# IllyaArtemchuk/Harmonies-Alphazero

Hardware: AMD Instinct MI355X
Metric: self-play env-steps/sec + games/sec @4096 boards, 1/2/4/8 GPUs; bit-exact vs CPU (higher is better)
Workload: dtype u64; 1 GPU; config2: 4096 concurrent boards/GPU, reset + rule-driven play to game end (legal mask, step, chance draws, final scoring); one step = 256 hz_play launches of 4096 boards; boards_per_gpu=4096, parallelism=shard1

## Files before the change

harmonies-alphazero_amd/csrc/hz_env.hip:

```cpp
#include <hip/hip_runtime.h>

#include <cstdio>
#include <cstdlib>
#include <cstring>

#include "../../include/hz_abi.h"
#include "hz_device.hpp"
#include "hz_encode.hpp"
#include "hz_host.hpp"

using namespace hz;
using namespace hz_host;

struct P2Draw {
  int32_t *tag;
  int32_t *k;
  uint64_t *q;
  uint64_t *bag;
  int32_t *c;
};
struct P2Mid {
  int32_t *tag;
  uint64_t *st;
  uint64_t *q;
  int32_t *i;
};

#ifndef HZ_P2_NDRAW
#define HZ_P2_NDRAW 5
#endif
#ifndef HZ_P2_NPLAY
#define HZ_P2_NPLAY 5
#endif
constexpr int kP2Draw = HZ_P2_NDRAW;
constexpr int kP2Play = HZ_P2_NPLAY;
constexpr int kP2SDraw = 4;
constexpr int kP2SPlay = kP2SDraw + kP2Draw;
constexpr int kP2Stages = kP2SPlay + kP2Play;
constexpr int kP2Last = kP2Stages - 1;
constexpr int kP2Ring = kP2Play + 1;
constexpr int kP2Stream = kP2Stages;
static_assert(kP2Draw >= 2 && kP2Draw <= 5 && kP2Play >= 2 && kP2Play <= 5, "stage counts");

struct hz_env {
  DevBufs bufs, p2_bufs, ar_bufs;
  int32_t n;
  uint64_t seed_base;
  hipStream_t stream;
  uint64_t *state;
  uint32_t *mt;
  int32_t *pos;
  int32_t *ply;
  int32_t *episode;
  uint64_t *seed;
  int seed_ahead;
  uint32_t *ahead_mt[2];
  int32_t *ahead_tag[2];
  uint64_t *ahead_pile[2];
  int32_t *ahead_cur[2];
  uint32_t *ahead_rule[2];
  int32_t *ep_final[2];
  size_t nrow;
  uint32_t *ring_mt[3];
  int32_t *ring_tag[3];
  uint64_t *ring_pile[3];
  int32_t *ring_cur[3];
  int32_t *ring_k1[3];
  int calls;
  int primed, slot_valid[2];
  int32_t *mt_src;
  int lazy;
  int ar_ahead;
  uint32_t *ar_mt;
  int32_t *ar_tag;
  uint64_t *ar_pile;
  int32_t *ar_cur;
  int32_t *ar_ep[2];
  int ar_calls, ar_primed;
  uint32_t *pw_words;
  int32_t *pw_tag;
  int pipeline;
  int calls2, primed2;
  int p2_cut[kP2Play - 1];
  int p2_dcut[kP2Draw + 1];
  int p2_fell_lim;
  uint32_t *p2_s[kP2Stream];
  int32_t *p2_s_tag[kP2Stream];
  int32_t *p2_s_cur[kP2Stream];
  uint32_t *p2_p1h[2];
  int32_t *p2_p1t[2];
  uint32_t *p2_p2h[2];
  uint32_t *p2_p3h[2];
  P2Draw p2_x[kP2Draw - 1][2];
  P2Draw p2_pl[kP2Ring];
  P2Mid p2_m[kP2Play - 1][2];
  uint32_t *p2_h[kP2Ring];
  int32_t *p2_h_tag[kP2Ring];
  int32_t *p2_ep[2];
  int32_t *wait_err_own;
  int32_t *wait_err;
  int spin_limit;
};

#ifdef HZ_DIAG
__device__ uint64_t *g_stamps;
__device__ int g_role_only = -1;
#define HZ_STAMP(slot)                                                    \
  do {                                                                    \
    __builtin_amdgcn_sched_barrier(0);                                    \
    if (g_stamps) g_stamps[(size_t)b * 16 + (slot)] = __builtin_amdgcn_s_memtime(); \
    __builtin_amdgcn_sched_barrier(0);                                    \
  } while (0)
#ifndef HZ_DIAG_ROLES_ONLY
#define HZ_ACC(slot, t0)                                                  \
  do {                                                                    \
    __builtin_amdgcn_sched_barrier(0);                                    \
    uint64_t _t = __builtin_amdgcn_s_memtime();                           \
    acc##slot += _t - (t0);                                               \
    t0 = _t;                                                              \
    __builtin_amdgcn_sched_barrier(0);                                    \
  } while (0)
#else
#define HZ_ACC(slot, t0) \
  do {                   \
  } while (0)
#endif
#define HZ_PHASE(slot, t0, b)                                                                 \
  do {                                                                                        \
    __builtin_amdgcn_sched_barrier(0);                                                        \
    if (g_stamps) g_stamps[(size_t)(b) * 16 + (slot)] = __builtin_amdgcn_s_memtime() - (t0); \
// ... 387 lines not shown
    if (lane + 64 * k < kMT) to[lane + 64 * k] = v[k];
  if (lane == 0) mt_src[b] = -1;
}

static PlyWin ply_win(hz_env *e) { return PlyWin{e->pw_words, e->pw_tag, (long)e->nrow}; }

static int touch(hz_env *e) { return streams_touched<HipDev>(e) ? 0 : 1; }

static int materialize(hz_env *e) {
  if (!e->lazy) return 0;
  if (e->ar_mt)
    hipLaunchKernelGGL(k_mt_materialize_ar, dim3(e->n), dim3(64), 0, e->stream, e->mt, e->ar_mt, e->mt_src, e->n);
  hipLaunchKernelGGL(k_mt_materialize, dim3(e->n), dim3(64), 0, e->stream, e->mt, e->ahead_mt[0], e->ahead_mt[1],
                     e->mt_src, e->n);
  if (e->p2_s[0])
    hipLaunchKernelGGL(k_mt_materialize2, dim3(grid_for(e->n)), dim3(kStageThreads), kResetLds, e->stream, e->mt,
                       e->seed, e->pos, e->mt_src, e->n);
  e->lazy = 0;
  return launch_err();
}

static_assert(sizeof(((hz_env *)0)->p2_s) / sizeof(uint32_t *) == kP2Stream, "slot ring");

static int p2_clear_tags(hz_env *e) {
  const size_t bytes = e->nrow * sizeof(int32_t);
  auto c = [&](int32_t *t) { return hipMemsetAsync(t, 0xff, bytes, e->stream) != hipSuccess; };
  for (int k = 0; k < kP2Stream; k++)
    if (c(e->p2_s_tag[k])) return 1;
  for (int k = 0; k < 2; k++)
    if (c(e->p2_p1t[k])) return 1;
  for (int k = 0; k < kP2Draw - 1; k++)
    if (c(e->p2_x[k][0].tag) || c(e->p2_x[k][1].tag)) return 1;
  for (int k = 0; k < kP2Ring; k++)
    if (c(e->p2_pl[k].tag) || c(e->p2_h_tag[k])) return 1;
  for (int k = 0; k < kP2Play - 1; k++)
    if (c(e->p2_m[k][0].tag) || c(e->p2_m[k][1].tag)) return 1;
  return 0;
}

static int alloc_p2(hz_env *e) {
  if (e->p2_s[0]) return 0;
  const size_t nr = e->nrow;
  DevBufs &o = e->p2_bufs;
  for (int k = 0; k < kP2Stream; k++) {
    o.get(e->p2_s[k], nr * kMT * 4);
    o.get(e->p2_s_tag[k], nr * 4);
    o.get(e->p2_s_cur[k], (kAheadDraws + 1) * nr * 4);
  }
  auto md = [&](P2Draw &d) {
    o.get(d.tag, nr * 4);
    o.get(d.k, nr * 4);
    o.get(d.q, kAheadWords * nr * 8);
    o.get(d.bag, nr * 8);
    o.get(d.c, nr * 4);
  };
  for (int k = 0; k < kP2Draw - 1; k++) md(e->p2_x[k][0]), md(e->p2_x[k][1]);
  for (int k = 0; k < kP2Ring; k++) {
    md(e->p2_pl[k]);
    o.get(e->p2_h[k], kRulePlies * nr * 4);
    o.get(e->p2_h_tag[k], nr * 4);
  }
  for (int k = 0; k < kP2Play - 1; k++)
    for (int j = 0; j < 2; j++) {
      P2Mid &mm = e->p2_m[k][j];
      o.get(mm.tag, nr * 4);
      o.get(mm.st, 6 * nr * 8);
      o.get(mm.q, 4 * nr * 8);
      o.get(mm.i, 3 * nr * 4);
    }
  for (int k = 0; k < 2; k++) {
    o.get(e->p2_p1h[k], nr * 4);
    o.get(e->p2_p1t[k], nr * 4);
    o.get(e->p2_p2h[k], 4 * nr * 4);
    o.get(e->p2_p3h[k], 4 * nr * 4);
    o.get(e->p2_ep[k], nr * 4);
  }
  if (!o.ok || p2_clear_tags(e)) {
    o.release();
    return 1;
  }
  e->primed2 = 0;
  return 0;
}

static int launch_play2(hz_env *e, int32_t max_plies, int32_t *games_done, int32_t *steps_done) {
  if (alloc_p2(e)) return 1;
  const int c = e->calls2, r = c & 1, w = r ^ 1;
  if (!e->primed2) {
    if (hipMemcpyAsync(e->p2_ep[w], e->episode, (size_t)e->n * sizeof(int32_t), hipMemcpyDeviceToDevice,
                       e->stream))
      return 1;
    e->primed2 = 1;
  }
  P2Args a{};
  a.st = e->state;
  a.mt = e->mt;
  a.pos = e->pos;
  a.ply = e->ply;
  a.episode = e->episode;
  a.seed = e->seed;
  a.n = e->n;
  a.max_plies = max_plies;
  a.err = e->wait_err;
  a.spin = e->spin_limit;
  a.seed_base = e->seed_base;
  a.nrow = (long)e->nrow;
  a.games_done = games_done;
  a.steps_done = steps_done;
  a.mt_src = e->mt_src;
  a.win_tag = e->pw_tag;
  a.ep_in = e->p2_ep[w];
  a.ep_out = e->p2_ep[r];
  auto sl = [c](int s) { return ((c - s) % kP2Stream + kP2Stream) % kP2Stream; };
  for (int s = 1; s < kP2SDraw; s++) {
    a.s_mt[s] = e->p2_s[sl(s)];
    a.s_tag[s] = e->p2_s_tag[sl(s)];
  }
  a.s_idx_last = sl(kP2Last);
  a.p1h_w = e->p2_p1h[r];
  a.p1t_w = e->p2_p1t[r];
  a.p2h_w = e->p2_p2h[r];
  a.p3h_w = e->p2_p3h[r];
  a.seed_tag[0] = e->p2_p1t[w];
  a.seed_tag[1] = a.s_tag[2];
  a.seed_tag[2] = a.s_tag[3];
  a.seed_h[0] = e->p2_p1h[w];
  a.seed_h[1] = e->p2_p2h[w];
  a.seed_h[2] = e->p2_p3h[w];
  const int draws = e->seed_ahead;
  for (int k = 0; k < kP2Draw; k++) {
    P2DrawArgs &d = a.dr[k];
    const int s = kP2SDraw + k;
    d.slot = e->p2_s[sl(s)];
    d.stag = e->p2_s_tag[sl(s)];
    d.cur = e->p2_s_cur[sl(s)];
    d.in = e->p2_x[k > 0 ? k - 1 : 0][w];
    d.out = k == kP2Draw - 1 ? e->p2_pl[c % kP2Ring] : e->p2_x[k][r];
    d.d0 = e->p2_dcut[k];
    d.d1 = k == kP2Draw - 1 ? draws : std::min(draws, e->p2_dcut[k + 1]);
  }
  a.h_w = e->p2_h[c % kP2Ring];
  a.ht_w = e->p2_h_tag[c % kP2Ring];
  for (int st = 0; st < kP2Play; st++) {
    P2PlayArgs &p = a.pp[st];
    const bool last = st == kP2Play - 1;
    const int s = kP2SPlay + st;
    const int k = (c + kP2Ring - 1 - st) % kP2Ring;
    p.ep = last ? e->episode : e->p2_ep[w];
    p.ep_off = last ? 0 : kP2Play - 1 - st;
    p.g0 = st > 0 ? e->p2_cut[st - 1] : 0;
    p.g_end = last ? max_plies : std::min(e->p2_cut[st], max_plies);
    p.fell_lim = e->p2_fell_lim;
    p.ptag = e->p2_pl[k].tag;
    p.pk = e->p2_pl[k].k;
    p.q = st > 0 ? e->p2_m[st - 1][w].q : e->p2_pl[k].q;
    p.h = e->p2_h[k];
    p.ht = e->p2_h_tag[k];
    p.slot = e->p2_s[sl(s)];
    p.cur = e->p2_s_cur[sl(s)];
    p.in = e->p2_m[st > 0 ? st - 1 : 0][w];
    p.out = e->p2_m[last ? 0 : st][r];
  }
  const int nblk = grid_for(e->n);
  hipLaunchKernelGGL(k_play2, dim3(4 * nblk), dim3(kStageThreads), kResetLds, e->stream, a, nblk);
  if (int err = launch_err()) return err;
  e->lazy = 1;
  e->calls2 = (c + 1) % (kP2Stream * kP2Ring * 2);
  e->primed = 0;
  e->ar_primed = 0;
  return 0;
}

extern "C" {

hz_env *hz_env_create(int32_t n_boards, uint64_t seed_base, void *stream) {
  if (n_boards <= 0) return nullptr;
  if (install_comp_table()) return nullptr;
  if (lds_opt_in<k_reset>(kResetLds) || lds_opt_in<k_rollout<false, false>>(kResetLds) ||
      lds_opt_in<k_rollout<false, true>>(kResetLds) || lds_opt_in<k_rollout<true, false>>(kResetLds) ||
      lds_opt_in<k_rollout<true, true>>(kResetLds) || lds_opt_in<k_play2>(kResetLds) ||
      lds_opt_in<k_mt_materialize2>(kResetLds))
    return nullptr;
  hz_env *e = new (std::nothrow) hz_env();
  if (!e) return nullptr;
  e->n = n_boards;
  e->seed_base = seed_base;
  e->stream = (hipStream_t)stream;
  const size_t n = (size_t)n_boards, nr = (n + kBlock - 1) / kBlock * kBlock, i32 = sizeof(int32_t);
  e->nrow = nr;
  DevBufs &o = e->bufs;
  o.get(e->state, n * 6 * sizeof(uint64_t), 0);
  o.get(e->mt, n * 624 * sizeof(uint32_t));
  o.get(e->pos, n * i32, 0);
  o.get(e->ply, n * i32, 0);
  o.get(e->episode, n * i32, 0);
  o.get(e->seed, n * sizeof(uint64_t), 0);
  o.get(e->mt_src, n * i32, 0xff);
  for (int k = 0; k < 2; k++) {
    o.get(e->ahead_mt[k], n * kMT * sizeof(uint32_t));
    o.get(e->ahead_tag[k], n * i32, 0xff);
    o.get(e->ahead_pile[k], n * kAheadWords * sizeof(uint64_t));
    o.get(e->ahead_cur[k], n * (kAheadDraws + 1) * i32);
    o.get(e->ahead_rule[k], nr * kRulePlies * sizeof(uint32_t));
    o.get(e->ep_final[k], n * i32);
  }
  for (int k = 0; k < kRing; k++) {
    o.get(e->ring_mt[k], nr * kMT * sizeof(uint32_t));
    o.get(e->ring_tag[k], nr * i32, 0xff);
    o.get(e->ring_pile[k], nr * 3 * sizeof(uint64_t));
    o.get(e->ring_cur[k], nr * (kD1Draws + 1) * i32);
    o.get(e->ring_k1[k], nr * i32);
  }
  o.get(e->pw_words, nr * kPlyWin * sizeof(uint32_t));
  o.get(e->pw_tag, nr * i32, 0xff);
  o.get(e->wait_err_own, i32, 0);
  e->seed_ahead = kAheadDraws;
  e->ar_ahead = env_pick("HZ_AR_AHEAD", 0, 1);
  e->pipeline = env_pick("HZ_PIPELINE", 1, 2);
  for (int k = 0; k < kP2Play - 1; k++) e->p2_cut[k] = kP2PCut[k];
  if constexpr (kP2Play == 4) env_cuts("HZ_P2_CUTS", e->p2_cut);
  else if constexpr (kP2Play == 5) env_cuts_n("HZ_P2_CUTS5", e->p2_cut, kP2Play - 1, 4, 1 << 20);
  for (int k = 0; k < kP2Draw; k++) e->p2_dcut[k] = kP2DCut[k];
  e->p2_dcut[kP2Draw] = kAheadDraws;
  if constexpr (kP2Draw == 5) {
    int dc[kP2Draw + 1];
    for (int k = 0; k <= kP2Draw; k++) dc[k] = e->p2_dcut[k];
    if (env_cuts_n("HZ_P2_DCUTS", dc + 1, kP2Draw - 1, 1, kAheadDraws - 1) &&
        cuts_gaps_within(dc, kP2Draw + 1, kP2StageDraws))
      for (int k = 0; k <= kP2Draw; k++) e->p2_dcut[k] = dc[k];
  }
  e->p2_fell_lim = env_clamped("HZ_P2_FELL_LIMIT", kP2Twist, 0, kP2Twist);
  e->wait_err = e->wait_err_own;
  e->spin_limit = kSpinLimitDefault;
  if (!o.ok || hipDeviceSynchronize() != hipSuccess) {
    hz_env_destroy(e);
    return nullptr;
  }
  return e;
}

void hz_env_destroy(hz_env *e) {
  if (!e) return;
  e->p2_bufs.release();
  e->ar_bufs.release();
  e->bufs.release();
  delete e;
}

int32_t hz_env_size(const hz_env *e) { return e ? e->n : -1; }

int hz_env_set_error_word(hz_env *e, int32_t *word) {
  if (!e) return -1;
  e->wait_err = word ? word : e->wait_err_own;
  return 0;
}

int hz_env_set_spin_limit(hz_env *e, int32_t limit) {
  if (!e || limit < 0) return -1;
  e->spin_limit = limit ? limit : kSpinLimitDefault;
  return 0;
}

int hz_env_set_pipeline(hz_env *e, int32_t pipeline) {
// ... 302 lines not shown
```

harmonies-alphazero_amd/csrc/hz_host.hpp:

```cpp
#pragma once

#include <atomic>
#include <cstddef>
#include <cstdint>
#include <cstdio>
#include <cstdlib>
#include <new>
#include <vector>

namespace hz_host {

inline int env_int(const char *name, int dflt) {
  const char *e = getenv(name);
  return e ? atoi(e) : dflt;
}

inline int env_pick(const char *name, int special, int otherwise) {
  return env_int(name, otherwise) == special ? special : otherwise;
}

inline int env_clamped(const char *name, int dflt, int lo, int hi) {
  const int v = env_int(name, dflt);
  return v < lo ? lo : v > hi ? hi : v;
}

inline void env_cuts(const char *name, int cut[3]) {
  const char *e = getenv(name);
  int c[3];
  if (e && sscanf(e, "%d,%d,%d", &c[0], &c[1], &c[2]) == 3 && c[0] > 0 && c[1] > c[0] && c[2] > c[1] &&
      c[0] % 4 == 0 && c[1] % 4 == 0 && c[2] % 4 == 0)
    for (int k = 0; k < 3; k++) cut[k] = c[k];
}

inline bool env_cuts_n(const char *name, int *cut, int n, int step, int hi) {
  const char *e = getenv(name);
  if (!e || n < 1 || n > 8 || step < 1) return false;
  int c[8];
  for (int k = 0; k < n; k++) {
    if (*e < '0' || *e > '9') return false;
    long v = 0;
    for (; *e >= '0' && *e <= '9'; e++)
      if ((v = v * 10 + (*e - '0')) > hi) return false;
    if (v < step || v % step || (k && v <= c[k - 1])) return false;
    c[k] = (int)v;
    if (*e++ != (k + 1 < n ? ',' : '\0')) return false;
  }
  for (int k = 0; k < n; k++) cut[k] = c[k];
  return true;
}

inline bool cuts_gaps_within(const int *cut, int n, int max_gap) {
  for (int k = 0; k + 1 < n; k++)
    if (cut[k + 1] - cut[k] > max_gap) return false;
  return true;
}

struct Setting {
  static constexpr int64_t kUnread = INT64_MIN;
  const char *name;
  int32_t dflt;
  std::atomic<int64_t> v{kUnread};
  int32_t get() {
    int64_t x = v.load(std::memory_order_relaxed);
    if (x == kUnread) {
      int64_t expect = kUnread;
      v.compare_exchange_strong(expect, (int64_t)env_int(name, dflt));
      x = v.load(std::memory_order_relaxed);
    }
    return (int32_t)x;
  }
  void set(int32_t x) { v.store(x, std::memory_order_relaxed); }
};

template <class Dev>
struct DevBufsT {
  struct Held {
    void *p;
    void *slot;
    void (*clear)(void *slot);
  };
  std::vector<Held> held;
  bool ok = true;

  template <class T>
  bool get(T *&p, size_t bytes) {
    if (!ok) return false;
// ... 68 lines not shown
```

harmonies-alphazero_amd/csrc/hz_play2.hpp:

```cpp
#pragma once

namespace {

#ifndef HZ_P2_ST_WT
#define HZ_P2_ST_WT 0
#endif
#ifndef HZ_P2_AUX
#define HZ_P2_AUX 16
#endif
#ifndef HZ_P2_STATIC_WIN
#define HZ_P2_STATIC_WIN 1
#endif
constexpr bool kP2StaticWin = HZ_P2_STATIC_WIN;

constexpr int kP2Win = 96;
constexpr int kP2WinRows = kP2Win + 24;
#ifndef HZ_P2_DCUT
#if HZ_P2_NDRAW == 5
#define HZ_P2_DCUT 0, 6, 11, 15, 19
#elif HZ_P2_NDRAW == 4
#define HZ_P2_DCUT 0, 7, 13, 18
#endif
#endif
constexpr int kP2DCut[kP2Draw] = {HZ_P2_DCUT};
constexpr int kP2StageDraws = 7;
#ifndef HZ_P2_PCUT
#if HZ_P2_NPLAY == 5
#define HZ_P2_PCUT 16, 32, 48, 64
#elif HZ_P2_NPLAY == 4
#define HZ_P2_PCUT 24, 40, 56
#endif
#endif
constexpr int kP2PCut[kP2Play - 1] = {HZ_P2_PCUT};
enum { kWvP1 = 8, kWvHash = 9, kWvPlay = 10, kWvIdle = 15 };
#ifndef HZ_P2_WAVES
#if HZ_P2_NDRAW == 5 && HZ_P2_NPLAY == 5
#define HZ_P2_WAVES 0, 1, 4, 9, 2, 3, 8, 10
#elif HZ_P2_NDRAW == 5
#define HZ_P2_WAVES 0, 1, 4, 9, 2, 3, 8, 15
#elif HZ_P2_NPLAY == 5
#define HZ_P2_WAVES 0, 1, 8, 9, 2, 3, 10, 15
#else
#define HZ_P2_WAVES 0, 1, 8, 9, 2, 3, 15, 15
#endif
#endif
constexpr int kP2Wave[8] = {HZ_P2_WAVES};
constexpr int p2_wave_count(int code) {
  int c = 0;
  for (int k = 0; k < 8; k++) c += kP2Wave[k] == code;
  return c;
}
constexpr bool p2_waves_ok() {
  for (int d = 0; d < 5; d++)
    if (p2_wave_count(d) != (d < kP2Draw ? 1 : 0)) return false;
  return p2_wave_count(kWvP1) == 1 && p2_wave_count(kWvHash) == 1 && p2_wave_count(kWvPlay) == (kP2Play == 5 ? 1 : 0);
}
static_assert(p2_waves_ok(), "HZ_P2_WAVES: every stage outside the seed and play blocks on exactly one wave");
constexpr int kP2MinPlies = 96;
#ifdef HZ_DIAG
constexpr int kP2Stamps = 48;
#define P2_PHASE(slot, t0)                                                                                       \
  do {                                                                                                           \
    __builtin_amdgcn_sched_barrier(0);                                                                           \
    if (g_stamps && b < a.n) g_stamps[(size_t)b * kP2Stamps + (slot)] = __builtin_amdgcn_s_memtime() - (t0); \
    __builtin_amdgcn_sched_barrier(0);                                                                           \
  } while (0)
#define P2_USE_V(x) asm volatile("" ::"v"(x))
#define P2_USE_S(x) asm volatile("" ::"s"(x))
#else
#define P2_PHASE(slot, t0) \
  do {                     \
  } while (0)
#define P2_USE_V(x) \
  do {              \
  } while (0)
#define P2_USE_S(x) \
  do {              \
  } while (0)
#endif
static_assert(4 * kP2WinRows * kWinStride * 4 <= (int)kResetLds, "a window per wave of a draw block");

struct P2DrawArgs {
  const uint32_t *slot;
  const int32_t *stag;
  int32_t *cur;
  P2Draw in, out;
  int d0, d1;
};
struct P2PlayArgs {
  const int32_t *ep;
  int ep_off;
  int g0;
  int g_end;
  int fell_lim;
  const int32_t *ptag, *pk;
  const uint64_t *q;
  const uint32_t *h;
  const int32_t *ht;
  uint32_t *slot;
  const int32_t *cur;
  P2Mid in, out;
};
struct P2Args {
  uint64_t *st;
  uint32_t *mt;
  int32_t *pos, *ply, *episode;
  uint64_t *seed;
  int n, max_plies;
  uint64_t seed_base;
  long nrow;
  int32_t *games_done, *steps_done, *mt_src;
  int32_t *win_tag;
  const int32_t *ep_in;
  int32_t *ep_out;
  P2DrawArgs dr[kP2Draw];
  P2PlayArgs pp[kP2Play];
  uint32_t *s_mt[kP2SDraw];
  int32_t *s_tag[kP2SDraw];
  const int32_t *seed_tag[3];
  const uint32_t *seed_h[3];
  int s_idx_last;
  uint32_t *p1h_w;
  int32_t *p1t_w;
  uint32_t *p2h_w;
  uint32_t *p3h_w;
  uint32_t *h_w;
  int32_t *ht_w;
  int32_t *err;
  int spin;
};

struct PlayDraw2 : PileScript {
  bool fell;
  MTR gm;
  const int32_t *cur_nd;
  __device__ __forceinline__ bool pair_pops() const { return d + 2 <= nd; }
  __device__ __forceinline__ bool lost() const { return fell && gm.over(); }
  __device__ __forceinline__ uint32_t draw_one(uint64_t misc) {
    if (d < nd) return pop();
    if (!fell) {
      gm = MTR(gm.w, gm.stride, *cur_nd, gm.lim);
      fell = true;
    }
    uint32_t p9;
    return draw_pile(misc, gm, p9) ? p9 : 0x1FFu;
  }
  __device__ __forceinline__ uint32_t operator()(uint64_t misc) { return take(misc, true); }
  __device__ __forceinline__ uint32_t take(uint64_t misc, bool want) {
    if (__all(!want || d < nd)) return pop_if(want);
    return want ? draw_one(misc) : 0x1FFu;
  }
};

template <class Draw>
__device__ __forceinline__ int p2_plies(State &s, Draw &draw, int g, int g_end, uint64_t rkey, const uint32_t *hs,
                                        size_t nr, const uint32_t *h0 = nullptr, int h0_g = -1) {
  const int g0 = g;
  auto hash = [&](int ply) -> uint32_t { return hs && ply < kRulePlies ? hs[(size_t)ply * nr] : rule_h32(rkey, ply); };
  const bool all_hs = __all(hs != nullptr);
  uint32_t hn[8];
// ... 67 lines not shown
  return *reinterpret_cast<const uint4 *>(p);
}
template <class T>
__device__ __forceinline__ T p2_at(const T *base, uint32_t off) {
  typedef __attribute__((address_space(1))) const char GlobalByte;
  typedef __attribute__((address_space(1))) const T GlobalT;
  return *(GlobalT *)((GlobalByte *)base + off);
}
template <class T>
__device__ __forceinline__ const T *p2_row(const T *base, size_t row_words) {
  const T *p = base + row_words;
  asm volatile("" : "+s"(p));
  return p;
}
__device__ __forceinline__ void p2_fence() { asm volatile("" ::: "memory"); }
__device__ __forceinline__ void p2_fence_use(int &x) { asm volatile("" : "+v"(x)::"memory"); }
template <class T>
__device__ __forceinline__ void p2_st(T *p, T v) {
  if constexpr (HZ_P2_AUX == 16 && HZ_P2_ST_WT) __hip_atomic_store(p, v, __ATOMIC_RELAXED, __HIP_MEMORY_SCOPE_AGENT);
  else *p = v;
}
__device__ __forceinline__ uint32_t p1_step(uint32_t t, uint32_t q, bool odd, uint32_t kA, uint32_t kB) {
  return (t ^ ((q ^ (q >> 30)) * 1664525U)) + (odd ? kA : kB);
}
__device__ __forceinline__ uint32_t p1_row1(uint32_t kA, uint32_t kB) {
  return p1_step(kInitGen.v[1], 19650218u, true, kA, kB);
}
__device__ __forceinline__ void p2_keys(uint64_t seed, uint32_t &kA, uint32_t &kB) {
  const uint32_t key0 = (uint32_t)seed, key1 = (uint32_t)(seed >> 32);
  kA = key0;
  kB = key1 ? key1 + 1u : key0;
}

typedef uint32_t u32x8 __attribute__((ext_vector_type(8)));
template <int Imm>
__device__ __forceinline__ u32x8 p1_load8(const uint32_t *tab, uint32_t off) {
  u32x8 t;
  asm volatile("s_load_dwordx8 %0, %1, %2 offset:%3" : "=&s"(t) : "s"(tab), "s"(off), "n"(Imm));
  return t;
}
__device__ __forceinline__ void p1_arrived(u32x8 &t) { asm volatile("s_waitcnt lgkmcnt(0)" : "+s"(t)); }
__device__ __forceinline__ uint32_t p1_steps8(const u32x8 &t, uint32_t prev, uint32_t kA, uint32_t kB) {
#pragma unroll
  for (int u = 0; u < 8; u++) prev = p1_step(t[u], prev, !(u & 1), kA, kB);
  return prev;
}
__device__ __forceinline__ void p2_p1(const P2Args &a, int b) {
  const int e = a.ep_in[b] + kP2Last;
  uint32_t kA, kB;
  p2_keys(episode_seed(a.seed_base, b, e), kA, kB);
  uint32_t prev = 19650218u;
  const uint32_t *tab = kInitGen.v + 1;
  static_assert(38 * 16 + 1 == 609 && 617 + 8 <= kMT + kInitGenPad, "the last group's read (rows 617-624) within the table's padding");
  u32x8 ta = p1_load8<0>(tab, 0), tb;
  p1_arrived(ta);
#pragma unroll 1
  for (uint32_t off = 0; off < 38 * 64; off += 64) {
    tb = p1_load8<32>(tab, off);
    __builtin_amdgcn_sched_barrier(0);
    prev = p1_steps8(ta, prev, kA, kB);
    __builtin_amdgcn_sched_barrier(0);
    p1_arrived(tb);
    ta = p1_load8<64>(tab, off);
    __builtin_amdgcn_sched_barrier(0);
    prev = p1_steps8(tb, prev, kA, kB);
    __builtin_amdgcn_sched_barrier(0);
    p1_arrived(ta);
  }
  tb = p1_load8<0>(tab, (617 - 1) * 4);
  prev = p1_steps8(ta, prev, kA, kB);
  p1_arrived(tb);
#pragma unroll
  for (int u = 0; u < 7; u++) prev = p1_step(tb[u], prev, !(u & 1), kA, kB);
  a.p1h_w[b] = p1_step(p1_row1(kA, kB), prev, false, kA, kB);
  a.p1t_w[b] = e * 8 + 2;
}

#ifndef HZ_P2_BEND
#define HZ_P2_BEND 433
#endif
#ifndef HZ_P2_AEND
#define HZ_P2_AEND 209
#endif
#ifndef HZ_P2_LEAN
#define HZ_P2_LEAN 1
#endif
#ifndef HZ_P2_TWIST
#define HZ_P2_TWIST 160
#endif
constexpr int kP2Twist = HZ_P2_TWIST;
constexpr int kP2Ahead = 0 | (kP2Twist << 16);
static_assert(kP2Twist % 8 == 0 && kP2Twist >= 64 && kP2Twist <= kAheadTwist, "the slot's twisted rows");
constexpr int kP2PartEnd = HZ_P2_LEAN ? kP2Twist + 1 : kAheadTwist + 1;
constexpr int p2_up8(int from, int x) { return x <= from ? from : from + 8 * ((x - from + 7) / 8); }
constexpr int p2_min(int a, int b) { return a < b ? a : b; }
constexpr int kP2aEnd = HZ_P2_AEND, kP2bEnd = HZ_P2_BEND;
static_assert(kP2bEnd > 399 && kP2bEnd + 64 < kMT && (kP2bEnd - kAheadTwist - 1) % 8 == 0, "P2b's final steps in groups of eight; rows 397, 398 P2b's");
static_assert(kP2aEnd > 11 && kP2aEnd <= kAheadTwist - 7 && (kAheadTwist + 1 - kP2aEnd) % 8 == 0, "P2b's part steps in groups of eight");
constexpr int kP2bDrop = HZ_P2_LEAN ? kAheadTwist + 1 + 8 * ((397 - kAheadTwist - 1) / 8) : kAheadTwist + 1;
struct P2Ahead {
  uint32_t cur[8];
  uint32_t iv[8];
  uint32_t last;
};
typedef __attribute__((address_space(4))) const uint32_t ConstWord;
__device__ __forceinline__ ConstWord *p2_table() {
  ConstWord *t = (ConstWord *)kInitGen.v;
// ... 73 lines not shown
#pragma unroll
    for (int u = 0; u < 8; u++) {
      h.cur[u] = nx[u];
      h.iv[u] = ivn[u];
    }
  }
}
template <int G, int G1, int Mode>
__device__ __forceinline__ void p2_tail(const P2Out &o, int lane, uint32_t &prev, P2Ahead &h) {
  static_assert(G1 - G >= 1 && G1 - G <= 8, "within the group ahead");
  [[maybe_unused]] const int soff = __builtin_amdgcn_readfirstlane((Mode == kP2Part ? G - 1 : G) * o.row_bytes);
#pragma unroll
  for (int i = G; i < G1; i++) {
    const uint32_t v = (h.cur[i - G] ^ ((prev ^ (prev >> 30)) * 1566083941U)) - (uint32_t)i;
    if constexpr (p2_mode_hbm(Mode)) o.put(Mode == kP2Part ? twist_part(prev, v) : v, soff, i - G);
    if (p2_mode_lds(Mode)) hz_lds[i * kLdsStride + lane] = v;
    prev = v;
  }
  h.last = h.cur[G1 - G - 1];
}

template <int K>
__device__ __forceinline__ void p2_third(const P2Args &a, int b0, int lane, int e, bool ok, const uint32_t (&hw)[4],
                                         int *s_prog) {
  const int b = b0 + lane;
  const bool act = b < a.n;
  const size_t nr = (size_t)a.nrow;
  if (K == 0 && act && !ok) a.s_tag[1][b] = -1;
  if (!__any(ok)) {
    if (K == 2) p2_publish(s_prog, kMT + 1);
    return;
  }
  uint32_t *slot = a.s_mt[1 + K];
  uint32_t kA, kB;
  p2_keys(episode_seed(a.seed_base, b, e), kA, kB);
  uint32_t prev, first1, row2, q;
  if (K == 0) {
    first1 = act ? hw[0] : 0u;
    prev = first1;
    q = p1_row1(kA, kB);
  } else {
    prev = act ? hw[0] : 0u;
    first1 = act ? hw[1] : 0u;
    row2 = act ? hw[2] : 0u;
    q = act ? hw[3] : 0u;
  }
  const __amdgpu_buffer_rsrc_t rs = p2_slot_rsrc(slot, b0, nr);
  const int row_bytes = __builtin_amdgcn_readfirstlane((int)(nr * 4));
  const P2Out o(rs, row_bytes, lane);
  ConstWord *tab = p2_table();
  P2Ahead h;
  if constexpr (K == 0) {
    q = p1_step(kInitGen.v[2], q, false, kA, kB);
    row2 = (q ^ ((prev ^ (prev >> 30)) * 1566083941U)) - 2U;
    prev = row2;
    p2_ahead_init<3>(tab, h, q, kA, kB);
    constexpr int G = 3 + 8 * ((kP2aEnd - 3) / 8), Gp = p2_min(G, p2_up8(3, kP2PartEnd));
    p2_span<3, Gp, kP2Part>(tab, o, prev, h, kA, kB, s_prog);
    p2_span<Gp, G, kP2None>(tab, o, prev, h, kA, kB, s_prog);
    p2_tail<G, kP2aEnd, (G < kP2PartEnd ? kP2Part : kP2None)>(o, lane, prev, h);
  } else if constexpr (K == 1) {
    p2_ahead_init<kP2aEnd>(tab, h, q, kA, kB);
    constexpr int E1 = kAheadTwist + 1, Pb = p2_min(E1, p2_up8(kP2aEnd, kP2PartEnd));
    p2_span<kP2aEnd, Pb, kP2Part>(tab, o, prev, h, kA, kB, s_prog);
    p2_span<Pb, E1, kP2None>(tab, o, prev, h, kA, kB, s_prog);
    if constexpr (!HZ_P2_LEAN)
      __builtin_amdgcn_raw_buffer_store_b32(prev, rs, lane * 4, kAheadTwist * row_bytes, HZ_P2_AUX);
    p2_span<E1, kP2bDrop, kP2None>(tab, o, prev, h, kA, kB, s_prog);
    p2_span<kP2bDrop, kP2bEnd, kP2Final>(tab, o, prev, h, kA, kB, s_prog);
  } else {
    const uint32_t f0 = act ? slot[(size_t)397 * nr + b] : 0u, f1 = act ? slot[(size_t)398 * nr + b] : 0u;
    p2_ahead_init<kP2bEnd>(tab, h, q, kA, kB);
    constexpr int G = kP2bEnd + 8 * ((kMT - kP2bEnd) / 8);
    constexpr int Keep = HZ_P2_LEAN ? kP2KeepLds : kP2Keep;
    constexpr int Kc = HZ_P2_LEAN ? p2_min(G, p2_up8(kP2bEnd, kP2Twist + 397)) : G;
    p2_span<kP2bEnd, Kc, Keep>(tab, o, prev, h, kA, kB, s_prog);
    p2_span<Kc, G, kP2None>(tab, o, prev, h, kA, kB, s_prog);
    p2_tail<G, kMT, (Kc == G ? Keep : kP2None)>(o, lane, prev, h);
    p2_publish(s_prog, kMT);
    const uint32_t row1 = (first1 ^ ((prev ^ (prev >> 30)) * 1566083941U)) - 1U;
    __builtin_amdgcn_raw_buffer_store_b32(f0 ^ twist_part(0x80000000u, row1), rs, lane * 4, 0, HZ_P2_AUX);
    __builtin_amdgcn_raw_buffer_store_b32(f1 ^ twist_part(row1, row2), rs, lane * 4, row_bytes, HZ_P2_AUX);
  }
  if (K < 2) {
    if (ok) {
      uint32_t *ho = K == 0 ? a.p2h_w : a.p3h_w;
      ho[b] = prev;
      ho[nr + b] = first1;
      ho[2 * nr + b] = row2;
      ho[3 * nr + b] = h.last;
      a.s_tag[1 + K][b] = e * 8 + 3 + K;
    }
  } else if (ok) {
    a.s_tag[3][b] = e * 8 + 5;
  }
}

#ifndef HZ_P2_TWGO
#define HZ_P2_TWGO 64
#endif
constexpr int kTwGo = HZ_P2_TWGO;
constexpr int kTwIters = kP2Twist / 4;
constexpr int kTwHbm = (kP2bEnd - 397 + 3) / 4;
__device__ __forceinline__ uint4 xor4(const uint4 &a, const uint4 &b) {
  return make_uint4(a.x ^ b.x, a.y ^ b.y, a.z ^ b.z, a.w ^ b.w);
}
__device__ __forceinline__ void p2_twist(const P2Args &a, int b0, int lane, bool any, int *s_prog) {
  if (!any) return;
  const size_t nr = (size_t)a.nrow;
  uint32_t *slot = a.s_mt[3];
  const int grp = lane >> 4, c4 = (lane & 15) * 4;
  uint32_t *col = slot + b0 + c4;
  auto row = [&](int r) { return p2_ld4(col + (size_t)r * nr); };
  const __amdgpu_buffer_rsrc_t rs = p2_slot_rsrc(slot, b0, nr);
  const int row_bytes = __builtin_amdgcn_readfirstlane((int)(nr * 4));
  auto store = [&](int r, const uint4 &v) {
    typedef uint32_t v4u __attribute__((ext_vector_type(4)));
    __builtin_amdgcn_raw_buffer_store_b128(v4u{v.x, v.y, v.z, v.w}, rs, c4 * 4 + r * row_bytes, 0, HZ_P2_AUX);
  };
  [[maybe_unused]] const int b = b0 + lane;
  HZ_DIAG_T0(tz);
  int have = kTwGo >= 0 ? p2_wait(s_prog, kP2bEnd + kTwGo, a.spin, a.err) : 0;
  P2_PHASE(35, tz);
  uint4 pt[kTwIters], fh[kTwHbm];
#pragma unroll
  for (int i = 0; i < kTwIters; i++) {
// ... 47 lines not shown
  int ep = p2_at(ep_in, (uint32_t)bc * 4u);
  const int tag = p2_at(tagp, (uint32_t)bc * 4u);
  uint32_t hw[4];
#pragma unroll
  for (int i = 0; i < 4; i++) hw[i] = p2_at(hrp[i], (uint32_t)hb * 4u);
  p2_fence_use(ep);
  const int e = act ? ep + kP2Last - 1 - k : 0;
  const bool ok = act && tag == e * 8 + 2 + k;
  __syncthreads();
  if (w == 0) p2_third<0>(a, b0, lane, e, ok, hw, &s_prog);
  else if (w == 1) p2_third<1>(a, b0, lane, e, ok, hw, &s_prog);
  else if (w == 2) p2_third<2>(a, b0, lane, e, ok, hw, &s_prog);
  else p2_twist(a, b0, lane, __any(ok), &s_prog);
}

__device__ __forceinline__ P2DrawArgs p2_draw_args(const P2Args &a, int stage, int &n, size_t &nr,
                                                   const int32_t *&ep_in) {
  const P2DrawArgs r = a.dr[stage];
  n = a.n;
  nr = (size_t)a.nrow;
  ep_in = a.ep_in;
  asm volatile("" ::"s"(r.slot), "s"(r.stag), "s"(r.cur), "s"(r.in.tag), "s"(r.in.k), "s"(r.in.q), "s"(r.in.bag),
               "s"(r.in.c), "s"(r.out.tag), "s"(r.out.k), "s"(r.out.q), "s"(r.out.bag), "s"(r.out.c), "s"(r.d0),
               "s"(r.d1), "s"(n), "s"(nr), "s"(ep_in));
  __builtin_amdgcn_sched_barrier(0);
  return r;
}
__device__ __forceinline__ P2PlayArgs p2_play_args(const P2Args &a, int st, int &n, size_t &nr, uint64_t &seed_base) {
  const P2PlayArgs r = a.pp[st];
  n = a.n;
  nr = (size_t)a.nrow;
  seed_base = a.seed_base;
  asm volatile("" ::"s"(r.ep), "s"(r.ep_off), "s"(r.g0), "s"(r.g_end), "s"(r.ptag), "s"(r.pk), "s"(r.q), "s"(r.h),
               "s"(r.ht), "s"(r.slot), "s"(r.cur), "s"(r.in.tag), "s"(r.in.st), "s"(r.in.q), "s"(r.in.i),
               "s"(r.out.tag), "s"(r.out.st), "s"(r.out.q), "s"(r.out.i), "s"(n), "s"(nr), "s"(seed_base),
               "s"(r.fell_lim));
  __builtin_amdgcn_sched_barrier(0);
  return r;
}
__device__ __forceinline__ int wave_min_i(int v) {
#pragma unroll
  for (int o = 32; o > 0; o >>= 1) v = min(v, __shfl_xor(v, o));
  return v;
}
__device__ __forceinline__ void p2_draw_stage(const P2Args &a, int b0, int lane, int stage, int base) {
  const int b = b0 + lane;
  HZ_DIAG_T0(t0);
  int n;
  size_t nr;
  const int32_t *ep_in;
  const P2DrawArgs r = p2_draw_args(a, stage, n, nr, ep_in);
  if (stage == 1) P2_PHASE(33, t0);
  const int d0 = r.d0, d1 = r.d1;
  const bool act = b < n;
  const uint32_t *slot = r.slot;
  int32_t *cur = r.cur + b;
  const P2Draw &in = r.in, &out = r.out;
  int k0 = 0, c0 = kP2Ahead;
  uint64_t bag = initial_bag(), q[kAheadWords] = {0, 0, 0, 0};
  constexpr int U = kP2Win / 4;
  const int c4 = (lane & 15) * 4;
  uint4 v[U];
  auto win_load = [&](int r0) {
#pragma unroll
    for (int u = 0; u < U; u++) {
      const int r = r0 + 4 * u + (lane >> 4);
      v[u] = p2_ld4(slot + (size_t)r * nr + b0 + c4);
// ... 21 lines not shown
  p2_fence();
  if (kP2StaticWin || stage == 0) win_load(rs);
  p2_fence_use(ep);
  if (stage == 1) {
    P2_USE_V(ep);
    P2_PHASE(34, t0);
  }
  const int e = act ? ep + kP2Last - kP2SDraw - stage : 0;
  bool ok = act && stag == e * 8 + 5;
  if (stage > 0) {
    k0 = ik;
    c0 = ic;
    bag = ibag;
#pragma unroll
    for (int i = 0; i < kAheadWords; i++) q[i] = iq[i];
    ok = ok && itag == e * 8 + stage;
  }
  if (stage == 1) {
    P2_USE_V((int)ok);
    P2_PHASE(26, t0);
  }
  bool draws = ok && k0 >= d0 && d0 < d1;
  int r0 = rs;
  if constexpr (kP2StaticWin) {
    draws = draws && (c0 & 0xFFFF) >= r0;
    win_store();
  } else {
    r0 = wave_min_i(draws ? (c0 & 0xFFFF) : kP2Twist) & ~3;
    if (r0 < kP2Twist) {
      if (stage > 0) win_load(r0);
      win_store();
    }
  }
  P2_PHASE(28 + stage, t0);
  if (!act) return;
  if (!ok) {
    out.tag[b] = -1;
    return;
  }
  if (stage == 0) cur[0] = kP2Ahead;
  int k = k0, cc = c0;
  if (draws) {
    const int lim = min(r0 + kP2Win, kP2Twist);
    StreamDraw<WinMT> d{WinMT(base - r0 * kWinStride + lane, c0, lim)};
#pragma unroll 1
    for (int i = d0; i < d1; i++) {
      if (d.m.pos >= lim) break;
      const uint32_t p9 = d(bag);
      if (d.m.pos > lim) break;
      apply_pile_fast(bag, p9);
      const int bit = 9 * i, wd = bit >> 6, off = bit & 63;
      const uint64_t lo9 = (uint64_t)p9 << off, hi9 = off > 55 ? (uint64_t)p9 >> (64 - off) : 0ull;
      q[0] |= wd == 0 ? lo9 : 0ull;
      q[1] |= wd == 1 ? lo9 : wd == 0 ? hi9 : 0ull;
      q[2] |= wd == 2 ? lo9 : wd == 1 ? hi9 : 0ull;
      q[3] |= wd == 3 ? lo9 : wd == 2 ? hi9 : 0ull;
      cc = d.m.cursor();
      p2_st(&cur[(size_t)(i + 1) * nr], cc);
      k = i + 1;
    }
  }
  p2_st(&out.k[b], k);
  p2_st(&out.c[b], cc);
  p2_st(&out.bag[b], bag);
#pragma unroll
  for (int i = 0; i < kAheadWords; i++) p2_st(&out.q[(size_t)i * nr + b], q[i]);
  p2_st(&out.tag[b], e * 8 + stage + 1);
}

__device__ __forceinline__ void p2_hashes(const P2Args &a, int b) {
  const size_t nr = (size_t)a.nrow;
  const int e = a.ep_in[b] + kP2Last - (kP2SPlay - 1);
  const uint64_t rk = rule_key(episode_seed(a.seed_base, b, e));
#pragma unroll 1
  for (int j = 0; j < kRulePlies; j++) p2_st(&a.h_w[(size_t)j * nr + b], rule_h32(rk, j));
  a.ht_w[b] = e;
}

__device__ __forceinline__ void p2_draw(const P2Args &a, int blk, int code) {
  const int tid = threadIdx.x, lane = tid & 63, w = tid >> 6;
  const int b0 = blk * kBlock;
  if (code < kP2Draw) {
    p2_draw_stage(a, b0, lane, code, w * kP2WinRows * kWinStride);
  } else if (code == kWvP1 && b0 + lane < a.n) {
    p2_p1(a, b0 + lane);
  } else if (code == kWvHash && b0 + lane < a.n) {
    p2_hashes(a, b0 + lane);
  }
}

__device__ __forceinline__ void p2_mid_put(const P2Mid &m, size_t nr, int b, const State &s, const PlayDraw2 &d, int g,
                                           int e) {
#pragma unroll
  for (int k = 0; k < 4; k++) p2_st(&m.st[(size_t)k * nr + b], s.pl[k]);
  p2_st(&m.st[4 * nr + b], s.piles);
  p2_st(&m.st[5 * nr + b], s.misc);
  p2_st(&m.q[b], d.q0);
  p2_st(&m.q[nr + b], d.q1);
  p2_st(&m.q[2 * nr + b], d.q2);
  p2_st(&m.q[3 * nr + b], d.q3);
  p2_st(&m.i[b], d.d);
  p2_st(&m.i[nr + b], g);
  p2_st(&m.i[2 * nr + b], d.fell ? d.gm.cursor() : -1);
  p2_st(&m.tag[b], e);
}

__device__ __forceinline__ void p2_play(const P2Args &a, int blk, int st, bool in_block) {
  __shared__ uint64_t s_lds_mask;
  const int tid = threadIdx.x, lane = tid & 63, w = tid >> 6;
  const int b0 = blk * kBlock, b = b0 + lane;
  HZ_DIAG_T0(t0);
  const bool last = st == kP2Play - 1;
  int n;
  size_t nr;
  uint64_t seed_base;
  const P2PlayArgs r = p2_play_args(a, st, n, nr, seed_base);
  const int fell_lim = r.fell_lim;
  if (last) P2_PHASE(38, t0);
  const bool act = b < n;
  const uint64_t actmask = __ballot(act);
  const int nb = n - b0 < kBlock ? n - b0 : kBlock;
  const int bc = min(b, n - 1), bi = st > 0 ? bc : b0;
  const uint32_t c4 = (uint32_t)bc * 4u, c8 = c4 * 2u, i4 = (uint32_t)bi * 4u, i8 = i4 * 2u;
  const bool h0_fits = r.g0 + 8 <= kRulePlies;
  const int h0_g = h0_fits ? r.g0 : -1;
  const size_t h0_row = h0_fits ? (size_t)r.g0 : 0;
  const uint64_t *qr[4], *str[6];
  const int32_t *ir[3];
  const uint32_t *hr[8];
#pragma unroll
  for (int k = 0; k < 4; k++) qr[k] = p2_row(r.q, (size_t)k * nr);
#pragma unroll
  for (int k = 0; k < 6; k++) str[k] = p2_row(r.in.st, (size_t)k * nr);
#pragma unroll
  for (int k = 0; k < 3; k++) ir[k] = p2_row(r.in.i, (size_t)k * nr);
#pragma unroll
  for (int j = 0; j < 8; j++) hr[j] = p2_row(r.h, (h0_row + j) * nr);
  p2_fence();
  int ep = p2_at(r.ep, c4);
  const int ptag = p2_at(r.ptag, c4), nd = p2_at(r.pk, c4), itag = p2_at(r.in.tag, i4), htg = p2_at(r.ht, c4);
  const int id = p2_at(ir[0], i4), ig = p2_at(ir[1], i4), ifc = p2_at(ir[2], i4);
  uint64_t sq[4], ist[6];
#pragma unroll
  for (int k = 0; k < 4; k++) sq[k] = p2_at(qr[k], c8);
#pragma unroll
  for (int k = 0; k < 6; k++) ist[k] = p2_at(str[k], i8);
  uint32_t h0[8];
#pragma unroll
  for (int j = 0; j < 8; j++) h0[j] = p2_at(hr[j], c4);
  p2_fence_use(ep);
  if (last) {
    P2_USE_V(ep);
    P2_PHASE(39, t0);
  }
  bool lds_used = false;
  if (act) {
    const int e = ep + r.ep_off;
    const P2Mid &mo = r.out;
    uint32_t *slot = r.slot + b;
    const int32_t *cur = r.cur + b;
    const int g_end = r.g_end;
    const uint64_t sd = episode_seed(seed_base, b, e), rk = rule_key(sd);
    const int mtag = st > 0 ? itag : e;
    const uint32_t *hs = htg == e ? r.h + b : nullptr;
    State s;
    int g = 0;
    PlayDraw2 draw{{sq[0], sq[1], sq[2], sq[3], 0, nd}, false, MTR(slot, (int)nr, 0, fell_lim), cur + (size_t)nd * nr};
    if (st > 0) {
#pragma unroll
      for (int k = 0; k < 4; k++) s.pl[k] = ist[k];
      s.piles = ist[4];
      s.misc = ist[5];
      g = ig;
      draw.d = id;
      draw.fell = ifc >= 0;
      draw.gm = MTR(slot, (int)nr, ifc >= 0 ? ifc : 0, fell_lim);
    }
    bool prep = ptag == e * 8 + kP2Draw && mtag == e;
    if (last) {
      P2_USE_V((int)prep);
      P2_PHASE(42, t0);
    }
    if (prep) {
      if (st == 0) {
        if (__all(nd >= 5)) draw.scripted_reset(s);
        else reset_state(s, draw);
      }
      P2_PHASE(16 + 2 * st, t0);
      g += p2_plies(s, draw, g, g_end, rk, hs, nr, h0, h0_g);
      P2_PHASE(17 + 2 * st, t0);
      if (draw.lost()) prep = false;
    }
    if (!last) {
      if (prep) p2_mid_put(mo, nr, b, s, draw, g, e);
      else mo.tag[b] = -1;
    } else {
      int cursor, src;
      if (prep) {
        cursor = draw.fell ? draw.gm.cursor() : cur[(size_t)draw.d * nr];
        src = 2 + a.s_idx_last;
      } else {
        mt_seed(hz_lds + lane, kLdsStride, sd);
        PlayDraw fb{{0, 0, 0, 0, 0, 0}, LdsMT(lane, kMTSeeded), false, false, MT(nullptr, 0), nullptr};
        reset_state(s, fb);
        g = p2_plies(s, fb, 0, a.max_plies, rk, nullptr, nr);
        cursor = fb.m.cursor();
        src = -1;
        lds_used = true;
      }
      a.episode[b] = e + 1;
      if (score_pending(s.misc)) finish_game(s);
// ... 82 lines not shown
```

Baseline: 24.75 billion env-steps/s.

## Fold rule-hash table generation into seed stages and add sixth draw stage

Removes the separate hash wave and its tag buffers. The rule-hash rows are now written in slices inside the existing seed stages (P1, P2/P3 hashes, final seed), and each slot gets its own hash table that travels with the slot ring. This frees a wave for a sixth draw stage with new draw cuts, and play stages no longer load or check a hash tag because the table is assumed valid for the slot. In exchange the seed stages do more work, the wave schedule changes, and correctness now depends on the slot ring always keeping the hash rows in step with the episode.

```diff
diff --git a/harmonies-alphazero_amd/csrc/hz_env.hip b/harmonies-alphazero_amd/csrc/hz_env.hip
--- a/harmonies-alphazero_amd/csrc/hz_env.hip
+++ b/harmonies-alphazero_amd/csrc/hz_env.hip
@@ -27,7 +27,7 @@
 };
 
 #ifndef HZ_P2_NDRAW
-#define HZ_P2_NDRAW 5
+#define HZ_P2_NDRAW 6
 #endif
 #ifndef HZ_P2_NPLAY
 #define HZ_P2_NPLAY 5
@@ -40,7 +40,7 @@
 constexpr int kP2Last = kP2Stages - 1;
 constexpr int kP2Ring = kP2Play + 1;
 constexpr int kP2Stream = kP2Stages;
-static_assert(kP2Draw >= 2 && kP2Draw <= 5 && kP2Play >= 2 && kP2Play <= 5, "stage counts");
+static_assert(kP2Draw >= 2 && kP2Draw <= 6 && kP2Play >= 2 && kP2Play <= 5, "stage counts");
 
 struct hz_env {
   DevBufs bufs, p2_bufs, ar_bufs;
@@ -94,8 +94,7 @@
   P2Draw p2_x[kP2Draw - 1][2];
   P2Draw p2_pl[kP2Ring];
   P2Mid p2_m[kP2Play - 1][2];
-  uint32_t *p2_h[kP2Ring];
-  int32_t *p2_h_tag[kP2Ring];
+  uint32_t *p2_h[kP2Stream];
   int32_t *p2_ep[2];
   int32_t *wait_err_own;
   int32_t *wait_err;
@@ -549,7 +548,7 @@
   for (int k = 0; k < kP2Draw - 1; k++)
     if (c(e->p2_x[k][0].tag) || c(e->p2_x[k][1].tag)) return 1;
   for (int k = 0; k < kP2Ring; k++)
-    if (c(e->p2_pl[k].tag) || c(e->p2_h_tag[k])) return 1;
+    if (c(e->p2_pl[k].tag)) return 1;
   for (int k = 0; k < kP2Play - 1; k++)
     if (c(e->p2_m[k][0].tag) || c(e->p2_m[k][1].tag)) return 1;
   return 0;
@@ -563,6 +562,7 @@
     o.get(e->p2_s[k], nr * kMT * 4);
     o.get(e->p2_s_tag[k], nr * 4);
     o.get(e->p2_s_cur[k], (kAheadDraws + 1) * nr * 4);
+    o.get(e->p2_h[k], kRulePlies * nr * 4);
   }
   auto md = [&](P2Draw &d) {
     o.get(d.tag, nr * 4);
@@ -574,8 +574,6 @@
   for (int k = 0; k < kP2Draw - 1; k++) md(e->p2_x[k][0]), md(e->p2_x[k][1]);
   for (int k = 0; k < kP2Ring; k++) {
     md(e->p2_pl[k]);
-    o.get(e->p2_h[k], kRulePlies * nr * 4);
-    o.get(e->p2_h_tag[k], nr * 4);
   }
   for (int k = 0; k < kP2Play - 1; k++)
     for (int j = 0; j < 2; j++) {
@@ -633,6 +631,7 @@
     a.s_mt[s] = e->p2_s[sl(s)];
     a.s_tag[s] = e->p2_s_tag[sl(s)];
   }
+  for (int s = 0; s < kP2SDraw; s++) a.s_h[s] = e->p2_h[sl(s)];
   a.s_idx_last = sl(kP2Last);
   a.p1h_w = e->p2_p1h[r];
   a.p1t_w = e->p2_p1t[r];
@@ -656,8 +655,6 @@
     d.d0 = e->p2_dcut[k];
     d.d1 = k == kP2Draw - 1 ? draws : std::min(draws, e->p2_dcut[k + 1]);
   }
-  a.h_w = e->p2_h[c % kP2Ring];
-  a.ht_w = e->p2_h_tag[c % kP2Ring];
   for (int st = 0; st < kP2Play; st++) {
     P2PlayArgs &p = a.pp[st];
     const bool last = st == kP2Play - 1;
@@ -671,8 +668,7 @@
     p.ptag = e->p2_pl[k].tag;
     p.pk = e->p2_pl[k].k;
     p.q = st > 0 ? e->p2_m[st - 1][w].q : e->p2_pl[k].q;
-    p.h = e->p2_h[k];
-    p.ht = e->p2_h_tag[k];
+    p.h = e->p2_h[sl(s)];
     p.slot = e->p2_s[sl(s)];
     p.cur = e->p2_s_cur[sl(s)];
     p.in = e->p2_m[st > 0 ? st - 1 : 0][w];
@@ -739,13 +735,7 @@
   else if constexpr (kP2Play == 5) env_cuts_n("HZ_P2_CUTS5", e->p2_cut, kP2Play - 1, 4, 1 << 20);
   for (int k = 0; k < kP2Draw; k++) e->p2_dcut[k] = kP2DCut[k];
   e->p2_dcut[kP2Draw] = kAheadDraws;
-  if constexpr (kP2Draw == 5) {
-    int dc[kP2Draw + 1];
-    for (int k = 0; k <= kP2Draw; k++) dc[k] = e->p2_dcut[k];
-    if (env_cuts_n("HZ_P2_DCUTS", dc + 1, kP2Draw - 1, 1, kAheadDraws - 1) &&
-        cuts_gaps_within(dc, kP2Draw + 1, kP2StageDraws))
-      for (int k = 0; k <= kP2Draw; k++) e->p2_dcut[k] = dc[k];
-  }
+  if constexpr (kP2Draw >= 5) env_p2_dcuts("HZ_P2_DCUTS", e->p2_dcut, kP2Draw, kAheadDraws, kP2StageDraws);
   e->p2_fell_lim = env_clamped("HZ_P2_FELL_LIMIT", kP2Twist, 0, kP2Twist);
   e->wait_err = e->wait_err_own;
   e->spin_limit = kSpinLimitDefault;
diff --git a/harmonies-alphazero_amd/csrc/hz_host.hpp b/harmonies-alphazero_amd/csrc/hz_host.hpp
--- a/harmonies-alphazero_amd/csrc/hz_host.hpp
+++ b/harmonies-alphazero_amd/csrc/hz_host.hpp
@@ -52,6 +52,21 @@
 inline bool cuts_gaps_within(const int *cut, int n, int max_gap) {
   for (int k = 0; k + 1 < n; k++)
     if (cut[k + 1] - cut[k] > max_gap) return false;
+  return true;
+}
+
+inline bool env_p2_dcuts(const char *name, int *dcut, int ndraw, int draws, int max_gap) {
+  if (ndraw < 2 || ndraw > 8) return false;
+  int dc[9];
+  for (int k = 0; k <= ndraw; k++) dc[k] = dcut[k];
+  bool got = ndraw == 6 && env_cuts_n(name, dc + 1, 5, 1, draws);
+  if (!got) {
+    const int n = ndraw == 6 ? 4 : ndraw - 1;
+    got = env_cuts_n(name, dc + 1, n, 1, draws - 1);
+    if (got && ndraw == 6 && dc[5] < dc[4]) dc[5] = dc[4];
+  }
+  if (!got || !cuts_gaps_within(dc, ndraw + 1, max_gap)) return false;
+  for (int k = 0; k <= ndraw; k++) dcut[k] = dc[k];
   return true;
 }
 
diff --git a/harmonies-alphazero_amd/csrc/hz_play2.hpp b/harmonies-alphazero_amd/csrc/hz_play2.hpp
--- a/harmonies-alphazero_amd/csrc/hz_play2.hpp
+++ b/harmonies-alphazero_amd/csrc/hz_play2.hpp
@@ -16,7 +16,9 @@
 constexpr int kP2Win = 96;
 constexpr int kP2WinRows = kP2Win + 24;
 #ifndef HZ_P2_DCUT
-#if HZ_P2_NDRAW == 5
+#if HZ_P2_NDRAW == 6
+#define HZ_P2_DCUT 0, 5, 9, 13, 17, 20
+#elif HZ_P2_NDRAW == 5
 #define HZ_P2_DCUT 0, 6, 11, 15, 19
 #elif HZ_P2_NDRAW == 4
 #define HZ_P2_DCUT 0, 7, 13, 18
@@ -32,16 +34,20 @@
 #endif
 #endif
 constexpr int kP2PCut[kP2Play - 1] = {HZ_P2_PCUT};
-enum { kWvP1 = 8, kWvHash = 9, kWvPlay = 10, kWvIdle = 15 };
+enum { kWvP1 = 8, kWvPlay = 10, kWvIdle = 15 };
 #ifndef HZ_P2_WAVES
-#if HZ_P2_NDRAW == 5 && HZ_P2_NPLAY == 5
-#define HZ_P2_WAVES 0, 1, 4, 9, 2, 3, 8, 10
+#if HZ_P2_NDRAW == 6 && HZ_P2_NPLAY == 5
+#define HZ_P2_WAVES 0, 1, 4, 5, 2, 3, 8, 10
+#elif HZ_P2_NDRAW == 6
+#define HZ_P2_WAVES 0, 1, 4, 5, 2, 3, 8, 15
+#elif HZ_P2_NDRAW == 5 && HZ_P2_NPLAY == 5
+#define HZ_P2_WAVES 0, 1, 4, 15, 2, 3, 8, 10
 #elif HZ_P2_NDRAW == 5
-#define HZ_P2_WAVES 0, 1, 4, 9, 2, 3, 8, 15
+#define HZ_P2_WAVES 0, 1, 4, 15, 2, 3, 8, 15
 #elif HZ_P2_NPLAY == 5
-#define HZ_P2_WAVES 0, 1, 8, 9, 2, 3, 10, 15
+#define HZ_P2_WAVES 0, 1, 8, 15, 2, 3, 10, 15
 #else
-#define HZ_P2_WAVES 0, 1, 8, 9, 2, 3, 15, 15
+#define HZ_P2_WAVES 0, 1, 8, 15, 2, 3, 15, 15
 #endif
 #endif
 constexpr int kP2Wave[8] = {HZ_P2_WAVES};
@@ -51,10 +57,18 @@
   return c;
 }
 constexpr bool p2_waves_ok() {
-  for (int d = 0; d < 5; d++)
+  for (int d = 0; d < 6; d++)
     if (p2_wave_count(d) != (d < kP2Draw ? 1 : 0)) return false;
-  return p2_wave_count(kWvP1) == 1 && p2_wave_count(kWvHash) == 1 && p2_wave_count(kWvPlay) == (kP2Play == 5 ? 1 : 0);
-}
+  return p2_wave_count(kWvP1) == 1 && p2_wave_count(kWvPlay) == (kP2Play == 5 ? 1 : 0);
+}
+#ifndef HZ_P2_HSPLIT
+#define HZ_P2_HSPLIT 24, 24, 52
+#endif
+constexpr int kP2HashSplit[3] = {HZ_P2_HSPLIT};
+constexpr int kP2HashCut[5] = {0, kP2HashSplit[0], kP2HashSplit[1], kP2HashSplit[2], kRulePlies};
+static_assert(0 <= kP2HashCut[1] && kP2HashCut[1] <= kP2HashCut[2] && kP2HashCut[2] <= kP2HashCut[3] &&
+                  kP2HashCut[3] <= kRulePlies,
+              "HZ_P2_HSPLIT: non-decreasing rows within the table");
 static_assert(p2_waves_ok(), "HZ_P2_WAVES: every stage outside the seed and play blocks on exactly one wave");
 constexpr int kP2MinPlies = 96;
 #ifdef HZ_DIAG
@@ -96,7 +110,6 @@
   const int32_t *ptag, *pk;
   const uint64_t *q;
   const uint32_t *h;
-  const int32_t *ht;
   uint32_t *slot;
   const int32_t *cur;
   P2Mid in, out;
@@ -124,8 +137,7 @@
   int32_t *p1t_w;
   uint32_t *p2h_w;
   uint32_t *p3h_w;
-  uint32_t *h_w;
-  int32_t *ht_w;
+  uint32_t *s_h[kP2SDraw];
   int32_t *err;
   int spin;
 };
@@ -259,6 +271,20 @@
   kB = key1 ? key1 + 1u : key0;
 }
 
+template <int S>
+__device__ __forceinline__ void p2_hash_rows(const P2Args &a, int b, uint64_t seed) {
+  constexpr int J0 = kP2HashCut[S], J1 = kP2HashCut[S + 1];
+  if constexpr (J0 < J1) {
+    __builtin_amdgcn_sched_barrier(0);
+    const size_t nr = (size_t)a.nrow;
+    const uint64_t rk = rule_key(seed);
+    uint32_t *h = a.s_h[S] + (size_t)J0 * nr + b;
+#pragma unroll 1
+    for (int j = J0; j < J1; j++, h += nr) p2_st(h, rule_h32(rk, j));
+    __builtin_amdgcn_sched_barrier(0);
+  }
+}
+
 typedef uint32_t u32x8 __attribute__((ext_vector_type(8)));
 template <int Imm>
 __device__ __forceinline__ u32x8 p1_load8(const uint32_t *tab, uint32_t off) {
@@ -274,8 +300,9 @@
 }
 __device__ __forceinline__ void p2_p1(const P2Args &a, int b) {
   const int e = a.ep_in[b] + kP2Last;
+  const uint64_t seed = episode_seed(a.seed_base, b, e);
   uint32_t kA, kB;
-  p2_keys(episode_seed(a.seed_base, b, e), kA, kB);
+  p2_keys(seed, kA, kB);
   uint32_t prev = 19650218u;
   const uint32_t *tab = kInitGen.v + 1;
   static_assert(38 * 16 + 1 == 609 && 617 + 8 <= kMT + kInitGenPad, "the last group's read (rows 617-624) within the table's padding");
@@ -300,6 +327,7 @@
 #pragma unroll
   for (int u = 0; u < 7; u++) prev = p1_step(tb[u], prev, !(u & 1), kA, kB);
   a.p1h_w[b] = p1_step(p1_row1(kA, kB), prev, false, kA, kB);
+  p2_hash_rows<0>(a, b, seed);
   a.p1t_w[b] = e * 8 + 2;
 }
 
@@ -439,8 +467,9 @@
     return;
   }
   uint32_t *slot = a.s_mt[1 + K];
+  const uint64_t seed = episode_seed(a.seed_base, b, e);
   uint32_t kA, kB;
-  p2_keys(episode_seed(a.seed_base, b, e), kA, kB);
+  p2_keys(seed, kA, kB);
   uint32_t prev, first1, row2, q;
   if (K == 0) {
     first1 = act ? hw[0] : 0u;
@@ -496,9 +525,11 @@
       ho[nr + b] = first1;
       ho[2 * nr + b] = row2;
       ho[3 * nr + b] = h.last;
+      p2_hash_rows<1 + K>(a, b, seed);
       a.s_tag[1 + K][b] = e * 8 + 3 + K;
     }
   } else if (ok) {
+    p2_hash_rows<3>(a, b, seed);
     a.s_tag[3][b] = e * 8 + 5;
   }
 }
@@ -612,7 +643,7 @@
   nr = (size_t)a.nrow;
   seed_base = a.seed_base;
   asm volatile("" ::"s"(r.ep), "s"(r.ep_off), "s"(r.g0), "s"(r.g_end), "s"(r.ptag), "s"(r.pk), "s"(r.q), "s"(r.h),
-               "s"(r.ht), "s"(r.slot), "s"(r.cur), "s"(r.in.tag), "s"(r.in.st), "s"(r.in.q), "s"(r.in.i),
+               "s"(r.slot), "s"(r.cur), "s"(r.in.tag), "s"(r.in.st), "s"(r.in.q), "s"(r.in.i),
                "s"(r.out.tag), "s"(r.out.st), "s"(r.out.q), "s"(r.out.i), "s"(n), "s"(nr), "s"(seed_base),
                "s"(r.fell_lim));
   __builtin_amdgcn_sched_barrier(0);
@@ -700,7 +731,7 @@
       win_store();
     }
   }
-  P2_PHASE(28 + stage, t0);
+  P2_PHASE(stage < 5 ? 28 + stage : 43, t0);
   if (!act) return;
   if (!ok) {
     out.tag[b] = -1;
@@ -736,15 +767,6 @@
   p2_st(&out.tag[b], e * 8 + stage + 1);
 }
 
-__device__ __forceinline__ void p2_hashes(const P2Args &a, int b) {
-  const size_t nr = (size_t)a.nrow;
-  const int e = a.ep_in[b] + kP2Last - (kP2SPlay - 1);
-  const uint64_t rk = rule_key(episode_seed(a.seed_base, b, e));
-#pragma unroll 1
-  for (int j = 0; j < kRulePlies; j++) p2_st(&a.h_w[(size_t)j * nr + b], rule_h32(rk, j));
-  a.ht_w[b] = e;
-}
-
 __device__ __forceinline__ void p2_draw(const P2Args &a, int blk, int code) {
   const int tid = threadIdx.x, lane = tid & 63, w = tid >> 6;
   const int b0 = blk * kBlock;
@@ -752,8 +774,6 @@
     p2_draw_stage(a, b0, lane, code, w * kP2WinRows * kWinStride);
   } else if (code == kWvP1 && b0 + lane < a.n) {
     p2_p1(a, b0 + lane);
-  } else if (code == kWvHash && b0 + lane < a.n) {
-    p2_hashes(a, b0 + lane);
   }
 }
 
@@ -806,7 +826,7 @@
   for (int j = 0; j < 8; j++) hr[j] = p2_row(r.h, (h0_row + j) * nr);
   p2_fence();
   int ep = p2_at(r.ep, c4);
-  const int ptag = p2_at(r.ptag, c4), nd = p2_at(r.pk, c4), itag = p2_at(r.in.tag, i4), htg = p2_at(r.ht, c4);
+  const int ptag = p2_at(r.ptag, c4), nd = p2_at(r.pk, c4), itag = p2_at(r.in.tag, i4);
   const int id = p2_at(ir[0], i4), ig = p2_at(ir[1], i4), ifc = p2_at(ir[2], i4);
   uint64_t sq[4], ist[6];
 #pragma unroll
@@ -830,7 +850,6 @@
     const int g_end = r.g_end;
     const uint64_t sd = episode_seed(seed_base, b, e), rk = rule_key(sd);
     const int mtag = st > 0 ? itag : e;
-    const uint32_t *hs = htg == e ? r.h + b : nullptr;
     State s;
     int g = 0;
     PlayDraw2 draw{{sq[0], sq[1], sq[2], sq[3], 0, nd}, false, MTR(slot, (int)nr, 0, fell_lim), cur + (size_t)nd * nr};
@@ -845,6 +864,7 @@
       draw.gm = MTR(slot, (int)nr, ifc >= 0 ? ifc : 0, fell_lim);
     }
     bool prep = ptag == e * 8 + kP2Draw && mtag == e;
+    const uint32_t *hs = r.h + b;
     if (last) {
       P2_USE_V((int)prep);
       P2_PHASE(42, t0);
```

New measurement: 26.01 billion env-steps/s, median of 6. 1.05x the previous value.
